# alibaba/VideoMV

Measured on AMD Instinct MI355X. Metric: denoise-steps/sec, t2v 320x512x24 (latent 24x40x64), CFG 9.0, 50-step DDIM schedule, higher is better.
Workload: dtype fp16; 1 GPU; t2v_infer.yaml UNetSD_T2VBase 1.413B, 24 views, latent 40x64, 77 ctx tokens, 1 sample per GPU (cond+uncond batched); parallelism=replicas x1

## Files before the change

videomv_amd/csrc/gemm_ff.hip:

```cpp
#include "gemm_glds_common.h"

using namespace vmvg;

namespace {

constexpr int FF_C = 320, FF_KS = FF_C / 32, FF_NT = FF_C / 16;
constexpr int FF_HC = 32;
constexpr int FF_W1_BYTES = 2 * FF_HC * FF_C * 2;
constexpr int FF_W2_BYTES = FF_C * FF_HC * 2;
constexpr int FF_STAGE = FF_W1_BYTES + FF_W2_BYTES;
constexpr int FF_B1_BYTES = 8 * FF_C * 4, FF_B2_BYTES = FF_C * 4;
constexpr int FF_LDS = 2 * FF_STAGE + FF_B1_BYTES + FF_B2_BYTES;
static_assert(FF_LDS <= 160 * 1024, "LDS budget");

constexpr int FF_PF1 = 1;
constexpr int FF_PF2 = 3;

VMV_DEV u32x4_t ff_swap16_xz_yw(u32x4_t v) {
    uint32_t x = v.x, y = v.y, z = v.z, w = v.w;
    asm("s_nop 3\n\tv_permlane16_swap_b32 %0, %2\n\tv_permlane16_swap_b32 %1, %3\n\ts_nop 1" : "+v"(x), "+v"(y), "+v"(z), "+v"(w));
    return u32x4_t{x, y, z, w};
}

__global__ __launch_bounds__(512, 1) void ff_fused_kernel(const VmvFfParams p) {
    VMV_KERNEL_ENTER();
    extern __shared__ __attribute__((aligned(16))) unsigned char smem[];
    const int tid = threadIdx.x;
    const int lane = tid & 63;
    const int wave = __builtin_amdgcn_readfirstlane(tid >> 6);
    const int frow = lane & 15, fgrp = lane >> 4;
    const int m_wave = blockIdx.x * 128 + wave * 16;
    const int nchunk = 4 * FF_C / FF_HC;

    const __amdgpu_buffer_rsrc_t x_rsrc = __builtin_amdgcn_make_buffer_rsrc(const_cast<void*>(p.x), 0, (uint32_t)p.M * (uint32_t)p.ldx * 2u, SRD_FLAGS);
    u32x4_t a[FF_KS];
    {
        const uint32_t vo = (uint32_t)((m_wave + frow) * p.ldx + 8 * fgrp) * 2u;
#pragma unroll
        for (int kk = 0; kk < FF_KS; ++kk) a[kk] = __builtin_amdgcn_raw_buffer_load_b128(x_rsrc, vo + (uint32_t)(kk * 64), 0, 0);
    }

    float* b1_lds = reinterpret_cast<float*>(smem + 2 * FF_STAGE);
    float* b2_lds = b1_lds + 8 * FF_C;
    {
        const __amdgpu_buffer_rsrc_t b1_rsrc = __builtin_amdgcn_make_buffer_rsrc(const_cast<float*>(p.b1), 0, p.b1 ? 8u * FF_C * 4u : 0u, SRD_FLAGS);
        const __amdgpu_buffer_rsrc_t b2_rsrc = __builtin_amdgcn_make_buffer_rsrc(const_cast<float*>(p.b2), 0, p.b2 ? FF_C * 4u : 0u, SRD_FLAGS);
        for (int q = wave; q * 256 < 8 * FF_C; q += 8)
            VMV_BLDS16(b1_rsrc, reinterpret_cast<unsigned char*>(b1_lds) + q * 1024, (uint32_t)(q * 256 + 4 * lane) * 4u, 0);
        if (wave < 2) VMV_BLDS16(b2_rsrc, reinterpret_cast<unsigned char*>(b2_lds) + wave * 1024, (uint32_t)(wave * 256 + 4 * lane) * 4u, 0);
    }
    const __amdgpu_buffer_rsrc_t w1_rsrc = __builtin_amdgcn_make_buffer_rsrc(const_cast<void*>(p.w1), 0, 8u * FF_C * FF_C * 2u, SRD_FLAGS);
    const __amdgpu_buffer_rsrc_t w2_rsrc = __builtin_amdgcn_make_buffer_rsrc(const_cast<void*>(p.w2), 0, (uint32_t)FF_C * 4u * FF_C * 2u, SRD_FLAGS);
    const int w2_slot = (lane & 3) ^ ((0x78 >> (2 * ((lane >> 4) & 3))) & 3);
    auto issue_chunk = [&](int c, int slot) {
        unsigned char* base = smem + slot * FF_STAGE;
        {
            const uint32_t so = (uint32_t)(c * 2 * FF_HC * FF_C) * 2u;
            int ln = lane;
            asm volatile("" : "+v"(ln));
#pragma unroll
            for (int q = 0; q < 5; ++q) {
                const int u = wave * 320 + q * 64 + ln;
                const int r = u / 40, s = u - r * 40;
                VMV_BLDS16(w1_rsrc, base + wave * 5120 + q * 1024, (uint32_t)(r * FF_C + (s ^ ((r >> 1) & 7)) * 8) * 2u, so);
            }
        }
        {
            const uint32_t so = (uint32_t)(c * FF_HC) * 2u;
            for (int t = wave; t < 20; t += 8)
                VMV_BLDS16(w2_rsrc, base + FF_W1_BYTES + t * 1024, (uint32_t)((16 * t + (lane >> 2)) * (4 * FF_C) + w2_slot * 8) * 2u, so);
        }
    };
    issue_chunk(0, 0);

    if (p.ln_eps > 0.f) {
        const float inv_k = 1.0f / (float)FF_C;
        float s1 = 0.f;
#pragma unroll
        for (int kk = 0; kk < FF_KS; ++kk) {
            elem_dot2c(s1, a[kk].x, VMV_ELEM_ONE2); elem_dot2c(s1, a[kk].y, VMV_ELEM_ONE2);
            elem_dot2c(s1, a[kk].z, VMV_ELEM_ONE2); elem_dot2c(s1, a[kk].w, VMV_ELEM_ONE2);
        }
        asm volatile("s_nop 4" : "+v"(s1));
        const float mean = xor16_32_sum(s1) * inv_k;
        float s2 = 0.f;
#pragma unroll
        for (int kk = 0; kk < FF_KS; ++kk) {
            const uint32_t w4[4] = {a[kk].x, a[kk].y, a[kk].z, a[kk].w};
#pragma unroll
            for (int e = 0; e < 4; ++e) {
                const float d0 = elem_lo(w4[e]) - mean, d1 = elem_hi(w4[e]) - mean;
                s2 = fmaf(d0, d0, s2); s2 = fmaf(d1, d1, s2);
            }
        }
        const float rstd = __builtin_amdgcn_rsqf(xor16_32_sum(s2) * inv_k + p.ln_eps);
        const float nm = -mean * rstd;
#pragma unroll
        for (int kk = 0; kk < FF_KS; ++kk) asm volatile("" : "+v"(a[kk].x), "+v"(a[kk].y), "+v"(a[kk].z), "+v"(a[kk].w));
#pragma unroll
        for (int kk = 0; kk < FF_KS; ++kk) {
            a[kk].x = pack_elem2(fmaf(elem_lo(a[kk].x), rstd, nm), fmaf(elem_hi(a[kk].x), rstd, nm));
            a[kk].y = pack_elem2(fmaf(elem_lo(a[kk].y), rstd, nm), fmaf(elem_hi(a[kk].y), rstd, nm));
            a[kk].z = pack_elem2(fmaf(elem_lo(a[kk].z), rstd, nm), fmaf(elem_hi(a[kk].z), rstd, nm));
            a[kk].w = pack_elem2(fmaf(elem_lo(a[kk].w), rstd, nm), fmaf(elem_hi(a[kk].w), rstd, nm));
        }
    }

    f32x4_t out[FF_NT];
#pragma unroll
    for (int j = 0; j < FF_NT; ++j) out[j] = f32x4_t{0.f, 0.f, 0.f, 0.f};

    const int fsw = (frow >> 1) & 7;
    int foff[2];
#pragma unroll
    for (int r = 0; r < 2; ++r) foff[r] = frow * 640 + (fgrp ^ (fsw & 3)) * 16 + ((r ^ (fsw >> 2)) - r) * 64;
    const int f2off = frow * 64 + (fgrp ^ ((0x78 >> (2 * ((frow >> 2) & 3))) & 3)) * 16;

    for (int c = 0; c < nchunk; ++c) {
        const int slot = c & 1;
        wait_vmcnt<0>();
        __builtin_amdgcn_s_waitcnt(0xc07f);
        __builtin_amdgcn_s_barrier();
        asm volatile("" ::: "memory");
        if (c + 1 < nchunk) issue_chunk(c + 1, slot ^ 1);
        const unsigned char* w1b = smem + slot * FF_STAGE;
        const unsigned char* w2b = w1b + FF_W1_BYTES + f2off;

        f32x4_t h1[4];
#pragma unroll
        for (int t = 0; t < 4; ++t) h1[t] = f32x4_t{0.f, 0.f, 0.f, 0.f};
        constexpr int PF1 = FF_PF1, NB1 = PF1 + 1;
        u32x4_t wf[NB1][4];
        auto rd1 = [&](const int kk, u32x4_t (&w)[4]) {
            const unsigned char* tp = w1b + foff[kk & 1] + 64 * kk;
#pragma unroll
            for (int t = 0; t < 4; ++t) w[t] = *reinterpret_cast<const u32x4_t*>(tp + t * (16 * 640));
        };
#pragma unroll
        for (int kk = 0; kk < PF1; ++kk) rd1(kk, wf[kk % NB1]);
#pragma unroll
        for (int kk = 0; kk < FF_KS; ++kk) {
            if (kk + PF1 < FF_KS) rd1(kk + PF1, wf[(kk + PF1) % NB1]);
            __builtin_amdgcn_sched_barrier(0);
#pragma unroll
            for (int t = 0; t < 4; ++t)
                h1[t] = VMV_MFMA16(__builtin_bit_cast(elem8_t, wf[kk % NB1][t]), __builtin_bit_cast(elem8_t, a[kk]), h1[t], 0, 0, 0);
            __builtin_amdgcn_sched_barrier(0);
        }
        constexpr int PF2 = FF_PF2, NB2 = PF2 + 1;
        u32x4_t w2f[NB2];
        auto rd2 = [&](const int j) -> u32x4_t { return *reinterpret_cast<const u32x4_t*>(w2b + j * (16 * 64)); };
#pragma unroll
        for (int j = 0; j < PF2; ++j) w2f[j % NB2] = rd2(j);
        u32x4_t hf;
        {
            const float* bb = b1_lds + c * 64 + 4 * fgrp;
            f32x4_t x0 = h1[0] + *reinterpret_cast<const f32x4_t*>(bb);
            const f32x4_t g0 = h1[1] + *reinterpret_cast<const f32x4_t*>(bb + 16);
            f32x4_t x1 = h1[2] + *reinterpret_cast<const f32x4_t*>(bb + 32);
            const f32x4_t g1 = h1[3] + *reinterpret_cast<const f32x4_t*>(bb + 48);
            x0.x *= gelu_erf_f(g0.x); x0.y *= gelu_erf_f(g0.y); x0.z *= gelu_erf_f(g0.z); x0.w *= gelu_erf_f(g0.w);
            x1.x *= gelu_erf_f(g1.x); x1.y *= gelu_erf_f(g1.y); x1.z *= gelu_erf_f(g1.z); x1.w *= gelu_erf_f(g1.w);
            hf.x = pack_elem2(x0.x, x0.y); hf.y = pack_elem2(x0.z, x0.w);
            hf.z = pack_elem2(x1.x, x1.y); hf.w = pack_elem2(x1.z, x1.w);
        }
#pragma unroll
        for (int j = 0; j < FF_NT; ++j) {
            if (j + PF2 < FF_NT) w2f[(j + PF2) % NB2] = rd2(j + PF2);
            __builtin_amdgcn_sched_barrier(0);
            out[j] = VMV_MFMA16(__builtin_bit_cast(elem8_t, w2f[j % NB2]), __builtin_bit_cast(elem8_t, hf), out[j], 0, 0, 0);
            __builtin_amdgcn_sched_barrier(0);
        }
    }

    const int lanecol = (fgrp & 1) * 16 + (fgrp >> 1) * 8;
    const __amdgpu_buffer_rsrc_t out_rsrc = __builtin_amdgcn_make_buffer_rsrc(p.out, 0, SRD_RECORDS, SRD_FLAGS);
    const __amdgpu_buffer_rsrc_t res_rsrc = __builtin_amdgcn_make_buffer_rsrc(const_cast<void*>(p.residual), 0, SRD_RECORDS, SRD_FLAGS);
    const bool ok = m_wave + frow < p.M;
    const uint32_t ovo = ok ? (uint32_t)((m_wave + frow) * p.ldo + lanecol) * 2u : OOB;
    const uint32_t rvo = (ok && p.residual) ? (uint32_t)((m_wave + frow) * p.ldr + lanecol) * 2u : OOB;
#pragma unroll
    for (int jp = 0; jp < FF_NT / 2; ++jp) {
        const u32x4_t rr = ff_swap16_xz_yw(__builtin_amdgcn_raw_buffer_load_b128(res_rsrc, rvo, (uint32_t)(32 * jp) * 2u, 0));
        f32x4_t v0 = out[2 * jp] + *reinterpret_cast<const f32x4_t*>(b2_lds + 32 * jp + 4 * fgrp);
        f32x4_t v1 = out[2 * jp + 1] + *reinterpret_cast<const f32x4_t*>(b2_lds + 32 * jp + 16 + 4 * fgrp);
        v0.x += elem_lo(rr.x); v0.y += elem_hi(rr.x); v0.z += elem_lo(rr.y); v0.w += elem_hi(rr.y);
        v1.x += elem_lo(rr.z); v1.y += elem_hi(rr.z); v1.z += elem_lo(rr.w); v1.w += elem_hi(rr.w);
        u32x4_t o;
        o.x = pack_elem2(v0.x, v0.y); o.y = pack_elem2(v0.z, v0.w);
        o.z = pack_elem2(v1.x, v1.y); o.w = pack_elem2(v1.z, v1.w);
        o = ff_swap16_xz_yw(o);
        __builtin_amdgcn_raw_buffer_store_b128(o, out_rsrc, ovo, (uint32_t)(32 * jp) * 2u, 0);
        asm volatile("s_nop 7" ::"v"(o.x), "v"(o.y), "v"(o.z), "v"(o.w) : "memory");
    }
}

}

extern "C" int vmv_ff_fused_ok(const VmvFfParams* pp) {
    if (!pp) return 0;
    const VmvFfParams& p = *pp;
    if (p.C != FF_C || p.M <= 0 || !p.x || !p.w1 || !p.w2 || !p.out) return 0;
    if ((p.ldx & 7) || (p.ldo & 7) || (p.residual && (p.ldr & 7))) return 0;
    if (!vmv_aligned16(p.x) || !vmv_aligned16(p.w1) || !vmv_aligned16(p.w2) || !vmv_aligned16(p.out) || (p.residual && !vmv_aligned16(p.residual))) return 0;
    if ((p.b1 && !vmv_aligned16(p.b1)) || (p.b2 && !vmv_aligned16(p.b2))) return 0;
    if ((long)(p.M + 128) * p.ldx * 2 >= (1L << 31) - 65536 || (long)(p.M + 128) * p.ldo * 2 >= (1L << 31) - 65536) return 0;
    if (p.residual && (long)(p.M + 128) * p.ldr * 2 >= (1L << 31) - 65536) return 0;
    return 1;
}

extern "C" int vmv_ff_fused(const VmvFfParams* pp, void* stream) {
    if (!pp) return VMV_ENULL;
    const VmvFfParams& p = *pp;
    if (!p.x || !p.w1 || !p.w2 || !p.out) return VMV_ENULL;
    if (p.C != FF_C || p.M <= 0) return VMV_EINVAL;
    if (!vmv_ff_fused_ok(pp)) return VMV_EALIGN;
    static std::atomic<unsigned long long> attr{0};
    if (const int rc_attr = vmv_lds_attr_once(attr, reinterpret_cast<const void*>(&ff_fused_kernel), FF_LDS)) return rc_attr;
    hipLaunchKernelGGL(ff_fused_kernel, dim3((p.M + 127) / 128), dim3(512), FF_LDS, reinterpret_cast<hipStream_t>(stream), p);
    return vmv_launch_status();
}
```

videomv_amd/unet_engine.py:

```python
import ctypes as C
import math
import os
from typing import Dict, List, Optional

import torch

from . import _lib as L
from . import ops
from . import packing as P



def block_plan(cfg):
    dim = cfg["dim"]
    dim_mult = list(cfg["dim_mult"])
    nrb = cfg["num_res_blocks"]
    hd = cfg["head_dim"]
    attn_scales = list(cfg["attn_scales"])
    enc_dims = [dim * u for u in [1] + dim_mult]
    dec_dims = [dim * u for u in [dim_mult[-1]] + dim_mult[::-1]]
    shortcut, scale = [], 1.0
    inp = [[("conv_in", "input_blocks.0.0", dict(cin=cfg["in_dim"], cout=dim)),
            ("tt", "input_blocks.0.1", dict(c=dim, heads=cfg["num_heads"], dh=hd))]]
    shortcut.append(dim)
    idx, out_dim = 1, dim
    for i, (in_dim, out_dim) in enumerate(zip(enc_dims[:-1], enc_dims[1:])):
        for j in range(nrb):
            p = f"input_blocks.{idx}"
            blk = [("res", f"{p}.0", dict(cin=in_dim, cout=out_dim))]
            if scale in attn_scales:
                blk.append(("st", f"{p}.1", dict(c=out_dim, heads=out_dim // hd, dh=hd, ctx=cfg["context_dim"])))
                blk.append(("tt", f"{p}.2", dict(c=out_dim, heads=out_dim // hd, dh=hd)))
            in_dim = out_dim
            inp.append(blk)
            shortcut.append(out_dim)
            idx += 1
            if i != len(dim_mult) - 1 and j == nrb - 1:
                inp.append([("down", f"input_blocks.{idx}", dict(c=out_dim))])
                shortcut.append(out_dim)
                scale /= 2.0
                idx += 1
    mid = [("res", "middle_block.0", dict(cin=out_dim, cout=out_dim)),
           ("st", "middle_block.1", dict(c=out_dim, heads=out_dim // hd, dh=hd, ctx=cfg["context_dim"])),
           ("tt", "middle_block.2", dict(c=out_dim, heads=out_dim // hd, dh=hd)),
           ("res", "middle_block.3", dict(cin=out_dim, cout=out_dim))]
    outb, idx = [], 0
    for i, (in_dim, out_dim) in enumerate(zip(dec_dims[:-1], dec_dims[1:])):
        for j in range(nrb + 1):
            p = f"output_blocks.{idx}"
            sc = shortcut.pop()
            blk = [("res", f"{p}.0", dict(cin=in_dim + sc, cout=out_dim, c_main=in_dim, c_skip=sc))]
            k = 1
            if scale in attn_scales:
                blk.append(("st", f"{p}.{k}", dict(c=out_dim, heads=out_dim // hd, dh=hd, ctx=1024)))
                blk.append(("tt", f"{p}.{k + 1}", dict(c=out_dim, heads=out_dim // hd, dh=hd)))
                k += 2
            in_dim = out_dim
            if i != len(dim_mult) - 1 and j == nrb:
                blk.append(("up", f"{p}.{k}", dict(c=out_dim)))
                scale *= 2.0
            outb.append(blk)
            idx += 1
    return inp, mid, outb


def _attn_shapes(p, c, inner, ctx):
    kv = inner if ctx is None else ctx
    return [(f"{p}.to_q.weight", (inner, c)), (f"{p}.to_k.weight", (inner, kv)), (f"{p}.to_v.weight", (inner, kv)),
            (f"{p}.to_out.0.weight", (c, inner)), (f"{p}.to_out.0.bias", (c,))]


def _tblock_shapes(p, inner, ctx):
    s = _attn_shapes(f"{p}.attn1", inner, inner, None)
    s += [(f"{p}.ff.net.0.proj.weight", (inner * 8, inner)), (f"{p}.ff.net.0.proj.bias", (inner * 8,)),
          (f"{p}.ff.net.2.weight", (inner, inner * 4)), (f"{p}.ff.net.2.bias", (inner,))]
    s += _attn_shapes(f"{p}.attn2", inner, inner, ctx)
    for n in ("norm1", "norm2", "norm3"):
        s += [(f"{p}.{n}.weight", (inner,)), (f"{p}.{n}.bias", (inner,))]
    return s


def param_shapes(cfg) -> "Dict[str, tuple]":
    dim = cfg["dim"]
    E = dim * 4
    s = [("time_embed.0.weight", (E, dim)), ("time_embed.0.bias", (E,)),
         ("time_embed.2.weight", (E, E)), ("time_embed.2.bias", (E,))]
    if cfg.get("use_camera_condition", False):
        s += [("camera_embedding.0.weight", (E, cfg["camera_dim"])), ("camera_embedding.0.bias", (E,)),
              ("camera_embedding.2.weight", (E, E)), ("camera_embedding.2.bias", (E,))]
    if cfg.get("use_fps_condition", False):
        s += [("fps_embedding.0.weight", (E, dim)), ("fps_embedding.0.bias", (E,)),
              ("fps_embedding.2.weight", (E, E)), ("fps_embedding.2.bias", (E,))]
    inp, mid, outb = block_plan(cfg)
    for blk in inp + [mid] + outb:
        for kind, p, m in blk:
            if kind == "conv_in":
                s += [(f"{p}.weight", (m["cout"], m["cin"], 3, 3)), (f"{p}.bias", (m["cout"],))]
            elif kind == "res":
                ci, co = m["cin"], m["cout"]
                s += [(f"{p}.in_layers.0.weight", (ci,)), (f"{p}.in_layers.0.bias", (ci,)),
                      (f"{p}.in_layers.2.weight", (co, ci, 3, 3)), (f"{p}.in_layers.2.bias", (co,)),
                      (f"{p}.emb_layers.1.weight", (co, E)), (f"{p}.emb_layers.1.bias", (co,)),
                      (f"{p}.out_layers.0.weight", (co,)), (f"{p}.out_layers.0.bias", (co,)),
                      (f"{p}.out_layers.3.weight", (co, co, 3, 3)), (f"{p}.out_layers.3.bias", (co,))]
                if ci != co:
                    s += [(f"{p}.skip_connection.weight", (co, ci, 1, 1)), (f"{p}.skip_connection.bias", (co,))]
                for name, ix in (("conv1", 2), ("conv2", 3), ("conv3", 3), ("conv4", 3)):
                    q = f"{p}.temopral_conv.{name}"
                    s += [(f"{q}.0.weight", (co,)), (f"{q}.0.bias", (co,)),
                          (f"{q}.{ix}.weight", (co, co, 3, 1, 1)), (f"{q}.{ix}.bias", (co,))]
            elif kind in ("st", "tt"):
                c = m["c"]
                inner = m["heads"] * m["dh"]
                s += [(f"{p}.norm.weight", (c,)), (f"{p}.norm.bias", (c,))]
                if kind == "st":
                    s += [(f"{p}.proj_in.weight", (inner, c)), (f"{p}.proj_in.bias", (inner,))]
                    s += _tblock_shapes(f"{p}.transformer_blocks.0", inner, m["ctx"])
                    s += [(f"{p}.proj_out.weight", (inner, c)), (f"{p}.proj_out.bias", (inner,))]
                else:
                    s += [(f"{p}.proj_in.weight", (inner, c, 1)), (f"{p}.proj_in.bias", (inner,))]
                    s += _tblock_shapes(f"{p}.transformer_blocks.0", inner, None)
                    s += [(f"{p}.proj_out.weight", (c, inner, 1)), (f"{p}.proj_out.bias", (c,))]
            elif kind == "down":
                s += [(f"{p}.op.weight", (m["c"], m["c"], 3, 3)), (f"{p}.op.bias", (m["c"],))]
            elif kind == "up":
                s += [(f"{p}.conv.weight", (m["c"], m["c"], 3, 3)), (f"{p}.conv.bias", (m["c"],))]
    s += [("out.0.weight", (dim,)), ("out.0.bias", (dim,)),
          ("out.2.weight", (cfg["out_dim"], dim, 3, 3)), ("out.2.bias", (cfg["out_dim"],))]
    return dict(s)


class Pool:

    def __init__(self, device):
        self.device = device
        self.free: Dict[int, List[torch.Tensor]] = {}
        self.all: List[torch.Tensor] = []
        self.bytes = 0

    def get(self, nbytes: int) -> torch.Tensor:
        nbytes = (int(nbytes) + 255) // 256 * 256
        lst = self.free.get(nbytes)
        if lst:
            return lst.pop()
        t = torch.empty(nbytes, dtype=torch.uint8, device=self.device)
        self.all.append(t)
        self.bytes += nbytes
        return t

    def put(self, t: torch.Tensor):
        self.free.setdefault(t.numel(), []).append(t)


class Act:
    __slots__ = ("buf", "rows", "C", "dtype")

    def __init__(self, buf, rows, C, dtype=None):
        self.buf, self.rows, self.C, self.dtype = buf, rows, C, dtype or L.elem()

    @property
    def ptr(self):
        return self.buf.data_ptr()

    def tensor(self) -> torch.Tensor:
        esz = 4 if self.dtype == torch.float32 else 2
        return self.buf[: self.rows * self.C * esz].view(self.dtype).view(self.rows, self.C)


class UNetEngine:
    def __init__(self, cfg: dict, weights: Dict[str, torch.Tensor], B: int, F: int, H: int, W: int, L_ctx: int,
                 device, n_t: int = 1, taps: Optional[dict] = None, comm=None, share_prefix: bool = False,
                 packed: Optional[dict] = None, eps_out: Optional[torch.Tensor] = None):
        self.share_prefix = bool(share_prefix) and B >= 2 and B % 2 == 0 and n_t == 1 and comm is None
        self.Bp = B // 2 if self.share_prefix else B
        self.comm = comm
        self.R = comm.world if comm is not None else 1
        self.rk = comm.rank if comm is not None else 0
        self.Fg = F
        if F % self.R:
            raise ValueError(f"{F} frames do not split over {self.R} ranks")
        F = F // self.R
        self.cfg, self.B, self.F, self.H, self.W, self.L = cfg, B, F, H, W, L_ctx
        self.B_ctx = B
        self.device = device
        self.breaks = []
        self.n_comm_ops, self.comm_bytes_in = 0, 0
        self.pool = Pool(device)
        self.S = ops.Stream(record=True)
        self.Sctx = ops.Stream(record=True)
        self._keepalive = []
        self._splitk = None
        self._gnws = torch.empty(4 << 20, dtype=torch.float32, device=device)
        self._gn_tot2 = torch.zeros(2, B * ops.GN_TOT, dtype=torch.int64, device=device)
        self._gn_zero = torch.zeros(2, B * ops.GN_TOT, dtype=torch.int64, device=device)
        self._gn_tot_k = 0
        self._gn_tot_all = torch.zeros(B * ops.GN_TOT * self.R, dtype=torch.int64, device=device) if comm is not None else None
        self.taps = taps
        self.n_t = n_t
        self.dim = cfg["dim"]
        self.E = self.dim * 4
        self.inp, self.mid, self.outb = block_plan(cfg)
        self.fold_ln = os.environ.get("VMV_FOLD_LN", "1") != "0"
        self.ln_inline = os.environ.get("VMV_LN_INLINE", "0") == "1"
        self.ff_fused = os.environ.get("VMV_FF_FUSED", "0") == "1" and self.fold_ln
        self.tqa = os.environ.get("VMV_TQA", "1") != "0"
        self.use_graph, self._replays, self.graph_nodes = os.environ.get("VMV_GRAPH", "0") == "1", 0, 0
        self.fp_temporal = os.environ.get("VMV_FP_TEMPORAL", "switch")
        if self.fp_temporal not in ("switch", "kv_gather"):
            raise ValueError("VMV_FP_TEMPORAL must be 'switch' or 'kv_gather'")
        if packed is not None and packed.get("fold_ln") == self.fold_ln and packed.get("device") == str(device):
            for k, v in packed.items():
                if k not in ("fold_ln", "device"):
                    setattr(self, k, v)
        else:
            self._pack(weights)
        self.packed = dict(fold_ln=self.fold_ln, device=str(device), w=self.w, has_cam=self.has_cam, has_fps=self.has_fps,
                           emb_off=self.emb_off, emb_total=self.emb_total, out_pad=self.out_pad)
        self._eps_out = eps_out
        self.n_tuned, self.n_ruled, self.n_stale = 0, 0, 0
        self.S.tuner = ops.make_tuner(self)
        self._static_inputs()
        self._build()
        if os.environ.get("VMV_AUTOTUNE", "0") == "1" and taps is None and str(device).startswith("cuda"):
            from . import autotune
            if autotune.autotune_engine(self, tag=f"B{B} F{self.Fg} {H}x{W} world{self.R}") > 0:
                self._rerecord()

    def _rerecord(self):
        dev = self.device
        self.B = self.B_ctx
        self.breaks, self.n_comm_ops, self.comm_bytes_in = [], 0, 0
        self.pool = Pool(dev)
        self.S = ops.Stream(record=True)
        self.Sctx = ops.Stream(record=True)
        self._keepalive, self._splitk = [], None
        self._gn_tot2.zero_()
        self._gn_tot_k = 0
        self._replays, self.graph_nodes, self.n_tuned, self.n_ruled, self.n_stale = 0, 0, 0, 0, 0
        self.S.tuner = ops.make_tuner(self)
        self._static_inputs()
        self._build()

    def _pack(self, sd):
        dev = self.device
        w: Dict[str, torch.Tensor] = {}
        self.w = w

        def lin(key, bias=True):
            w[key + ".weight"] = P.pack_linear(sd[key + ".weight"], dev)
            if bias and (key + ".bias") in sd:
                w[key + ".bias"] = P.pack_bias(sd[key + ".bias"], dev)

        def norm(key):
            w[key + ".weight"] = P.f32(sd[key + ".weight"], dev)
            w[key + ".bias"] = P.f32(sd[key + ".bias"], dev)

        def folded(key, wt, b, nkey, geglu=False):
            if not self.fold_ln:
                return
            wf, bf, cs = P.fold_layernorm(wt, b, sd[nkey + ".weight"], sd[nkey + ".bias"])
            if geglu:
                wf, bf, cs = P.geglu_interleave(wf), P.geglu_interleave(bf), P.geglu_interleave(cs)
            w[key + ".ln.weight"] = P.pack_linear(wf, dev)
            w[key + ".ln.bias"] = P.pack_bias(bf, dev)
            w[key + ".ln.colsum"] = P.pack_bias(cs, dev)

        def tblock(p, temporal=False):
            for a in ("attn1", "attn2"):
                q = sd[f"{p}.{a}.to_q.weight"]
                k = sd[f"{p}.{a}.to_k.weight"]
                v = sd[f"{p}.{a}.to_v.weight"]
                nk = "norm1" if a == "attn1" else "norm2"
                if k.shape[1] == q.shape[1]:
                    if not self.fold_ln:
                        w[f"{p}.{a}.qkv"] = P.pack_linear(torch.cat([q, k, v], dim=0), dev)
                    folded(f"{p}.{a}.qkv", torch.cat([q, k, v], dim=0), None, f"{p}.{nk}")
                    if temporal and self.tqa and q.shape[1] == 320 and q.shape[0] % 64 == 0:
                        for sfx in ((".ln.weight", ".ln.bias", ".ln.colsum") if self.fold_ln else ("",)):
                            src = w[f"{p}.{a}.qkv{sfx}"]
                            w[f"{p}.{a}.qkv.hm{sfx}"] = P.qkv_head_major(src[: 3 * q.shape[0]]).contiguous()
                else:
                    if not self.fold_ln:
                        w[f"{p}.{a}.q"] = P.pack_linear(q, dev)
                    folded(f"{p}.{a}.q", q, None, f"{p}.{nk}")
                    w[f"{p}.{a}.kv"] = P.pack_linear(torch.cat([k, v], dim=0), dev)
                lin(f"{p}.{a}.to_out.0")
            if not self.fold_ln:
                w[f"{p}.ff.net.0.proj.weight"] = P.pack_linear(P.geglu_interleave(sd[f"{p}.ff.net.0.proj.weight"]), dev)
            w[f"{p}.ff.net.0.proj.bias"] = P.pack_bias(P.geglu_interleave(sd[f"{p}.ff.net.0.proj.bias"]), dev)
            folded(f"{p}.ff.net.0.proj", sd[f"{p}.ff.net.0.proj.weight"], sd[f"{p}.ff.net.0.proj.bias"], f"{p}.norm3", geglu=True)
            lin(f"{p}.ff.net.2")
            if self.fold_ln and sd[f"{p}.ff.net.2.weight"].shape[0] == 320:
                w[f"{p}.ff.net.2.weight.ffperm"] = P.pack_linear(P.ff_down_permute(sd[f"{p}.ff.net.2.weight"]), dev)
            for n in ("norm1", "norm2", "norm3"):
                norm(f"{p}.{n}")

        lin("time_embed.0"); lin("time_embed.2")
        self.has_cam = "camera_embedding.0.weight" in sd
        if self.has_cam:
            lin("camera_embedding.0"); lin("camera_embedding.2")
        self.has_fps = self.cfg.get("use_fps_condition", False) and "fps_embedding.0.weight" in sd
        if self.has_fps:
            lin("fps_embedding.0"); lin("fps_embedding.2")
        emb_w, emb_b, self.emb_off = [], [], {}
        off = 0
        for blk in self.inp + [self.mid] + self.outb:
            for kind, p, m in blk:
                if kind == "conv_in":
                    w[p + ".weight"] = P.pack_conv3x3(sd[p + ".weight"], dev)
                    w[p + ".bias"] = P.pack_bias(sd[p + ".bias"], dev)
                elif kind == "res":
                    norm(f"{p}.in_layers.0")
                    w[f"{p}.in_layers.2.weight"] = P.pack_conv3x3(sd[f"{p}.in_layers.2.weight"], dev)
                    w[f"{p}.in_layers.2.bias"] = P.pack_bias(sd[f"{p}.in_layers.2.bias"], dev)
                    emb_w.append(sd[f"{p}.emb_layers.1.weight"]); emb_b.append(sd[f"{p}.emb_layers.1.bias"])
                    self.emb_off[p] = off
                    off += m["cout"]
                    norm(f"{p}.out_layers.0")
                    w2 = sd[f"{p}.out_layers.3.weight"]
# ... 253 lines not shown
        T = B * F * h * w
        cout = m["cout"]
        geom = ops.Geom(OH=h, OW=w, IH=h, IW=w, stride=1, ups=0)
        h0 = self._gn(p + ".gn1", srcs, T, h * w, f"{p}.in_layers.0", 1e-5, True)
        h1 = self.act(T, cout)
        self._gemm(p + ".conv1", T, cout, ops.conv3x3_segs([(h0.ptr, h0.C, h0.C)]), f"{p}.in_layers.2.weight", h1,
                   bias=self.w[f"{p}.in_layers.2.bias"], geom=geom,
                   rowvec=self.emb_out.data_ptr() + 4 * self.emb_off[p], rowvec_div=h * w, rowvec_ld=self.emb_total)
        self.release(h0)
        h2 = self._gn(p + ".gn2", [h1], T, h * w, f"{p}.out_layers.0", 1e-5, True)
        self.release(h1)
        h3 = self.act(T, cout)
        segs = ops.conv3x3_segs([(h2.ptr, h2.C, h2.C)])
        if m["cin"] != cout:
            segs += ops.linear_segs([(s.ptr, s.C, s.C) for s in srcs])
            self._gemm(p + ".conv2+skip", T, cout, segs, f"{p}.conv2.weight", h3, bias=self.w[f"{p}.conv2.bias"], geom=geom)
        else:
            self._gemm(p + ".conv2", T, cout, segs, f"{p}.conv2.weight", h3, bias=self.w[f"{p}.conv2.bias"], geom=geom,
                       residual=srcs[0].ptr, ldr=srcs[0].C)
        self.release(h2)
        if self.comm is not None:
            h3 = self._switch(h3, h * w, to_pixel=True)
        tg = ops.Geom(F=self.Fg, P=(h * w) // self.R)
        cur = h3
        for i, name in enumerate(("conv1", "conv2", "conv3", "conv4")):
            q = f"{p}.temopral_conv.{name}"
            nxt = self.act(T, cout)
            last = i == 3
            if not self._tconv_folded(q, cur, T, F * h * w, nxt, tg, residual=h3.ptr if last else None, ldr=h3.C if last else 0):
                g = self._gn(q + ".gn", [cur], T, F * h * w, f"{q}.0", 1e-5, True, all_frames=True)
                self._gemm(q, T, cout, ops.temporal_segs(g.ptr, g.C, g.C), f"{q}.weight", nxt, bias=self.w[f"{q}.bias"],
                           geom=tg, residual=h3.ptr if last else None, ldr=h3.C if last else 0)
                self.release(g)
            if cur is not h3:
                self.release(cur)
            cur = nxt
        self.release(h3)
        if self.comm is not None:
            cur = self._switch(cur, h * w, to_pixel=False)
        return cur

    def _tblock(self, p, a: Act, heads, temporal: bool, h, w, cross_ctx: bool, phase: str = "all", kv_gather: bool = False) -> Act:
        B, F = self.B, self.F
        T = a.rows
        inner = a.C
        hw = h * w
        scale = 64 ** -0.5

        if temporal and not kv_gather:
            hw, F = hw // self.R, self.Fg

        def maps(ld, col0=0):
            if temporal:
                return ops.seq_map(F * hw * ld, ld, hw * ld, inner=hw)
            return ops.seq_map(hw * ld, 0, ld, inner=1)

        n_outer = B * hw if temporal else B * F
        Nq = F if temporal else hw

        def fused_qkv_attn(tag, x: Act, normkey):
            hm = f"{p}.{tag}.qkv.hm"
            if not (temporal and not kv_gather and self.tqa and (hm + (".ln.weight" if self.fold_ln else "")) in self.w):
                return None
            ao = self.act(T, inner)
            geom = ops.Geom(F=F, P=hw)
            if self.fold_ln:
                gp = ops.gemm_params(T, 3 * inner, ops.linear_segs([(x.ptr, x.C, x.C)]), self.w[hm + ".ln.weight"], ao.ptr, ao.C,
                                     bias=self.w[hm + ".ln.bias"], colsum=self.w[hm + ".ln.colsum"], ln_eps=1e-5,
                                     epilogue=L.EPI_TATTN, epi_scale=scale, geom=geom)
                ln = None
            else:
                ln = self._ln(f"{p}.{tag}.qkv.ln", x, f"{p}.{normkey}")
                gp = ops.gemm_params(T, 3 * inner, ops.linear_segs([(ln.ptr, ln.C, ln.C)]), self.w[hm], ao.ptr, ao.C,
                                     epilogue=L.EPI_TATTN, epi_scale=scale, geom=geom)
            if not self.S.lib.vmv_gemm_tqa_ok(C.byref(gp)):
                self.release(ao)
                if ln is not None:
                    self.release(ln)
                return None
            self.S.gemm(gp, f"{p}.{tag}.qkv+attn")
            if ln is not None:
                self.release(ln)
            return ao

        def self_attn(tag, x: Act, normkey) -> Act:
            ao = fused_qkv_attn(tag, x, normkey)
            if ao is not None:
                y = self.act(T, inner)
                self._gemm(f"{p}.{tag}.out", T, inner, ops.linear_segs([(ao.ptr, ao.C, ao.C)]), f"{p}.{tag}.to_out.0.weight", y,
                           bias=self.w[f"{p}.{tag}.to_out.0.bias"], residual=x.ptr, ldr=x.C)
                self.release(ao)
                return y
            qkv = self.act(T, 3 * inner)
            self._ln_linear(f"{p}.{tag}.qkv", x, f"{p}.{normkey}", 3 * inner, f"{p}.{tag}.qkv", qkv)
            ao = self.act(T, inner)
            ld = 3 * inner
            if kv_gather:
                cv = inner // 8
                kvloc = self.act(T, 2 * inner)
                self.S.copy(ops.copy_params(qkv.ptr + 2 * inner, kvloc.ptr, T, 1, 1, 2 * cv, 3 * cv, 0), f"{p}.{tag}.kv.pack")
                kvall = self.act(self.R * T, 2 * inner)
                out_t, in_t = kvall.tensor().view(-1), kvloc.tensor().view(-1)
                self._collective(L.COMM_ALL_GATHER, out_t, in_t, f"{p}.{tag}.kv.gather")
                self.release(kvloc)
                qm = ops.seq_map(0, ld, hw * ld, inner=hw)
                km = ops.seq_map(0, 2 * inner, hw * 2 * inner, inner=hw)
                self.S.attention(ops.attn_params(qkv.ptr, kvall.ptr, kvall.ptr + 2 * inner, ao.ptr, qm, km, km,
                                                 ops.seq_map(0, inner, hw * inner, inner=hw), hw, heads, F, self.Fg, scale),
                                 f"{p}.{tag}.attn")
                self.release(kvall)
            else:
                self.S.attention(ops.attn_params(qkv.ptr, qkv.ptr + 2 * inner, qkv.ptr + 4 * inner, ao.ptr,
                                                 maps(ld), maps(ld), maps(ld), maps(inner), n_outer, heads, Nq, Nq, scale),
                                 f"{p}.{tag}.attn")
            self.release(qkv)
            y = self.act(T, inner)
            self._gemm(f"{p}.{tag}.out", T, inner, ops.linear_segs([(ao.ptr, ao.C, ao.C)]), f"{p}.{tag}.to_out.0.weight", y,
                       bias=self.w[f"{p}.{tag}.to_out.0.bias"], residual=x.ptr, ldr=x.C)
            self.release(ao)
            return y

        def cross_attn(tag, x: Act, normkey) -> Act:
            q = self.act(T, inner)
            self._ln_linear(f"{p}.{tag}.q", x, f"{p}.{normkey}", inner, f"{p}.{tag}.q", q)
            Lc = self.L
            Bc = self.B_ctx
            kvt = torch.empty(Bc * Lc, 2 * inner, dtype=L.elem(), device=self.device)
            self._keepalive.append(kvt)
            kv = Act(kvt.view(torch.uint8).view(-1), Bc * Lc, 2 * inner)
            cd = self.ctx_rows.shape[1]
            self._gemm(f"{p}.{tag}.kv", Bc * Lc, 2 * inner, ops.linear_segs([(self.ctx_rows.data_ptr(), cd, cd)]),
                       f"{p}.{tag}.kv", kv, stream=self.Sctx)
            ao = self.act(T, inner)
            kvm = ops.seq_map(Lc * 2 * inner, 0, 2 * inner, inner=1)
            self.S.attention(ops.attn_params(q.ptr, kv.ptr, kv.ptr + 2 * inner, ao.ptr, maps(inner), kvm, kvm, maps(inner),
                                             n_outer, heads, Nq, Lc, scale, kv_div=F), f"{p}.{tag}.attn")
            self.release(q)
            y = self.act(T, inner)
            self._gemm(f"{p}.{tag}.out", T, inner, ops.linear_segs([(ao.ptr, ao.C, ao.C)]), f"{p}.{tag}.to_out.0.weight", y,
                       bias=self.w[f"{p}.{tag}.to_out.0.bias"], residual=x.ptr, ldr=x.C)
            self.release(ao)
            return y

        if phase == "post":
            a1 = a
        else:
            a1 = self_attn("attn1", a, "norm1")
            if phase == "pre":
                return a1
        a2 = cross_attn("attn2", a1, "norm2") if cross_ctx else self_attn("attn2", a1, "norm2")
        if phase != "post":
            self.release(a1)
        a3 = self.act(T, inner)
        if self.ff_fused and f"{p}.ff.net.2.weight.ffperm" in self.w and T >= 16384:
            fp = ops.ff_params(T, inner, a2.ptr, a2.C, self.w[f"{p}.ff.net.0.proj.ln.weight"], self.w[f"{p}.ff.net.0.proj.ln.bias"],
                               self.w[f"{p}.ff.net.2.weight.ffperm"], self.w[f"{p}.ff.net.2.bias"], a3.ptr, a3.C,
                               residual=a2.ptr, ldr=a2.C, ln_eps=1e-5)
            if self.S.lib.vmv_ff_fused_ok(C.byref(fp)):
                self.S.ff(fp, f"{p}.ff.fused")
                self.release(a2)
                return a3
        ff = self.act(T, 4 * inner)
        self._ln_linear(f"{p}.ff.geglu", a2, f"{p}.norm3", 8 * inner, f"{p}.ff.net.0.proj.weight", ff,
                        bias=self.w[f"{p}.ff.net.0.proj.bias"], epilogue=L.EPI_GEGLU)
        self._gemm(f"{p}.ff.down", T, inner, ops.linear_segs([(ff.ptr, ff.C, ff.C)]), f"{p}.ff.net.2.weight", a3,
                   bias=self.w[f"{p}.ff.net.2.bias"], residual=a2.ptr, ldr=a2.C)
        self.release(ff); self.release(a2)
        return a3

    def _transformer(self, kind, p, m, x: Act, h, w, cut: bool = False) -> Act:
        B, F = self.B, self.F
        T = x.rows
        C = x.C
        inner = m["heads"] * m["dh"]
        if m["dh"] != 64:
            raise NotImplementedError("the HIP attention kernel is specialised for head_dim 64")
        temporal = kind == "tt"
        sharded = temporal and self.comm is not None
        kvg = sharded and self.fp_temporal == "kv_gather" and self.B == 1 and not cut
        if sharded and not kvg:
            x = self._switch(x, h * w, to_pixel=True, release_in=False)
        rps = (F * h * w) if temporal else (h * w)
        a = self.act(T, inner)
        if not self._gn_folded_proj_in(p, x, T, rps, a, temporal):
            n0 = self._gn(p + ".norm", [x], T, rps, f"{p}.norm", 1e-6, False, all_frames=temporal)
            self._gemm(p + ".proj_in", T, inner, ops.linear_segs([(n0.ptr, n0.C, n0.C)]), f"{p}.proj_in.weight", a,
                       bias=self.w[f"{p}.proj_in.bias"])
            self.release(n0)
        if cut:
            assert not temporal and self.B == self.Bp
            a1 = self._tblock(f"{p}.transformer_blocks.0", a, m["heads"], temporal, h, w, cross_ctx=True, phase="pre")
            self.release(a)
            self.B = self.B_ctx
            x_full, a1_full = self._replicate(x, p + ".share.x"), self._replicate(a1, p + ".share.a1")
            self.release(a1)
            x, T = x_full, x_full.rows
            a3 = self._tblock(f"{p}.transformer_blocks.0", a1_full, m["heads"], temporal, h, w, cross_ctx=True, phase="post")
            self.release(a1_full)
        else:
            a3 = self._tblock(f"{p}.transformer_blocks.0", a, m["heads"], temporal, h, w, cross_ctx=not temporal, kv_gather=kvg)
            self.release(a)
        y = self.act(T, C)
        self._gemm(p + ".proj_out", T, C, ops.linear_segs([(a3.ptr, a3.C, a3.C)]), f"{p}.proj_out.weight", y,
                   bias=self.w[f"{p}.proj_out.bias"], residual=x.ptr, ldr=x.C)
        self.release(a3)
        if cut:
            self.release(x)
        if sharded and not kvg:
            self.release(x)
            y = self._switch(y, h * w, to_pixel=False)
        return y

    def _run_block(self, blk, srcs: List[Act], h, w):
        x = None
        for kind, p, m in blk:
            ins = srcs if x is None else [x]
            if kind == "conv_in":
                T_in = self.B * self.F * h * w
                y = self.act(T_in, m["cout"])
                self._gemm(p, T_in, m["cout"], ops.conv3x3_segs([(self.x_rows.data_ptr(), self.cin_pad, self.cin_pad)]),
                           p + ".weight", y, bias=self.w[p + ".bias"], geom=ops.Geom(OH=h, OW=w, IH=h, IW=w))
            elif kind == "res":
                y = self._res_block(p, m, ins, h, w)
            elif kind in ("st", "tt"):
                y = self._transformer(kind, p, m, ins[0], h, w, cut=(kind == "st" and self.B != self.B_ctx))
            elif kind == "down":
                xin = ins[0]
                oh, ow = (h + 1) // 2, (w + 1) // 2
                T = self.B * self.F * oh * ow
                y = self.act(T, m["c"])
                self._gemm(p, T, m["c"], ops.conv3x3_segs([(xin.ptr, xin.C, xin.C)]), p + ".weight", y,
                           bias=self.w[p + ".bias"], geom=ops.Geom(OH=oh, OW=ow, IH=h, IW=w, stride=2))
                h, w = oh, ow
            elif kind == "up":
                xin = ins[0]
                oh, ow = h * 2, w * 2
                T = self.B * self.F * oh * ow
                y = self.act(T, m["c"])
                self._gemm(p, T, m["c"], ops.conv3x3_segs([(xin.ptr, xin.C, xin.C)]), p + ".weight", y,
                           bias=self.w[p + ".bias"], geom=ops.Geom(OH=oh, OW=ow, IH=h, IW=w, stride=1, ups=1))
                h, w = oh, ow
            else:
                raise ValueError(kind)
            if x is not None:
                self.release(x)
            x = y
        return x, h, w

    def _build(self):
        B, F = self.B, self.F
        S = self.S
        S.copy(ops.copy_params(self._gn_zero.data_ptr(), self._gn_tot2.data_ptr(), 1, 1, 1, self._gn_tot2.numel() // 2, 0, 0),
               "gn.totals.clear")
        self.n_emb_ops_start = S.nops
        e = Act(self.emb_silu.view(torch.uint8).view(-1), B * F, self.E)
        eo = Act(self.emb_out.view(torch.uint8).view(-1), B * F, self.emb_total, torch.float32)
        self._gemm("emb_all", B * F, self.emb_total, ops.linear_segs([(e.ptr, e.C, e.C)]), "emb_all.weight", eo,
                   bias=self.w["emb_all.bias"], out_fp32=True)
        h, w = self.H, self.W
        xs = []
        x = None
        share = self.share_prefix and len(self.inp) > 1 and any(k == "st" for k, _, _ in self.inp[1])
        if share:
            self.B = self.Bp
        for bi, blk in enumerate(self.inp):
            x, h, w = self._run_block(blk, [x] if x is not None else [], h, w)
            if share and bi == 0:
                x1 = x
                x_skip = self._replicate(x1, "share.skip0")
                xs.append((x_skip, h, w))
                if self.taps is not None:
                    self.taps[blk[0][1]] = (x_skip, h, w)
                continue
            if share and bi == 1:
                self.release(x1)
            xs.append((x, h, w))
            if self.taps is not None:
                self.taps[blk[0][1]] = (x, h, w)
        assert self.B == self.B_ctx
        x_last = x
        x, h, w = self._run_block(self.mid, [x], h, w)
        if self.taps is not None:
            self.taps["middle_block"] = (x, h, w)
        for blk in self.outb:
            skip, sh, sw = xs.pop()
            assert (sh, sw) == (h, w), (sh, sw, h, w)
            y, h, w = self._run_block(blk, [x, skip], h, w)
            if x is not skip:
                self.release(x)
            self.release(skip)
            x = y
            if self.taps is not None:
                self.taps[blk[0][1]] = (x, h, w)
        T = self.T0
        hn = self._gn("out.gn", [x], T, h * w, "out.0", 1e-5, True)
        self.release(x)
        eps = Act(self.eps_rows.view(torch.uint8).view(-1), T, self.out_pad, torch.float32)
        self._gemm("out.conv", T, self.out_pad, ops.conv3x3_segs([(hn.ptr, hn.C, hn.C)]), "out.2.weight", eps,
                   bias=self.w["out.2.bias"], geom=ops.Geom(OH=h, OW=w, IH=h, IW=w), out_fp32=True)
        self.release(hn)

    def set_context(self, y: torch.Tensor):
        self.ctx_rows.copy_(y.reshape(self.B * self.L, -1).to(L.elem()))
        self.context_updated()

    def context_updated(self):
        if self.Sctx.nops:
# ... 133 lines not shown
```

Baseline: 19.73 denoise-steps/s.

## Split fused FF wave work across wave pairs with software-pipelined down-projection

```diff
diff --git a/videomv_amd/csrc/gemm_ff.hip b/videomv_amd/csrc/gemm_ff.hip
--- a/videomv_amd/csrc/gemm_ff.hip
+++ b/videomv_amd/csrc/gemm_ff.hip
@@ -8,12 +8,14 @@
 constexpr int FF_HC = 32;
 constexpr int FF_W1_BYTES = 2 * FF_HC * FF_C * 2;
 constexpr int FF_W2_BYTES = FF_C * FF_HC * 2;
-constexpr int FF_STAGE = FF_W1_BYTES + FF_W2_BYTES;
-constexpr int FF_B1_BYTES = 8 * FF_C * 4, FF_B2_BYTES = FF_C * 4;
-constexpr int FF_LDS = 2 * FF_STAGE + FF_B1_BYTES + FF_B2_BYTES;
+constexpr int FF_B1_PIECE = 1024, FF_B2_BYTES = FF_C * 4;
+constexpr int FF_XCH_BYTES = 8 * 2 * 512;
+constexpr int FF_OFF_W2 = 2 * FF_W1_BYTES, FF_OFF_B1 = FF_OFF_W2 + 3 * FF_W2_BYTES, FF_OFF_B2 = FF_OFF_B1 + 2 * FF_B1_PIECE;
+constexpr int FF_OFF_XCH = FF_OFF_B2 + FF_B2_BYTES;
+constexpr int FF_LDS = FF_OFF_XCH + 2 * FF_XCH_BYTES;
 static_assert(FF_LDS <= 160 * 1024, "LDS budget");
 
-constexpr int FF_PF1 = 1;
+constexpr int FF_PF1 = 2;
 constexpr int FF_PF2 = 3;
 
 VMV_DEV u32x4_t ff_swap16_xz_yw(u32x4_t v) {
@@ -29,51 +31,50 @@
     const int lane = tid & 63;
     const int wave = __builtin_amdgcn_readfirstlane(tid >> 6);
     const int frow = lane & 15, fgrp = lane >> 4;
-    const int m_wave = blockIdx.x * 128 + wave * 16;
+    const int m_wave = blockIdx.x * 128 + (wave >> 1) * 32;
+    const int half = wave & 1;
     const int nchunk = 4 * FF_C / FF_HC;
 
     const __amdgpu_buffer_rsrc_t x_rsrc = __builtin_amdgcn_make_buffer_rsrc(const_cast<void*>(p.x), 0, (uint32_t)p.M * (uint32_t)p.ldx * 2u, SRD_FLAGS);
-    u32x4_t a[FF_KS];
+    u32x4_t a[2][FF_KS];
     {
-        const uint32_t vo = (uint32_t)((m_wave + frow) * p.ldx + 8 * fgrp) * 2u;
-#pragma unroll
-        for (int kk = 0; kk < FF_KS; ++kk) a[kk] = __builtin_amdgcn_raw_buffer_load_b128(x_rsrc, vo + (uint32_t)(kk * 64), 0, 0);
-    }
-
-    float* b1_lds = reinterpret_cast<float*>(smem + 2 * FF_STAGE);
-    float* b2_lds = b1_lds + 8 * FF_C;
+#pragma unroll
+        for (int rt = 0; rt < 2; ++rt) {
+        const uint32_t vo = (uint32_t)((m_wave + 16 * rt + frow) * p.ldx + 8 * fgrp) * 2u;
+#pragma unroll
+        for (int kk = 0; kk < FF_KS; ++kk) a[rt][kk] = __builtin_amdgcn_raw_buffer_load_b128(x_rsrc, vo + (uint32_t)(kk * 64), 0, 0);
+        }
+    }
+
+    float* b2_lds = reinterpret_cast<float*>(smem + FF_OFF_B2);
     {
-        const __amdgpu_buffer_rsrc_t b1_rsrc = __builtin_amdgcn_make_buffer_rsrc(const_cast<float*>(p.b1), 0, p.b1 ? 8u * FF_C * 4u : 0u, SRD_FLAGS);
         const __amdgpu_buffer_rsrc_t b2_rsrc = __builtin_amdgcn_make_buffer_rsrc(const_cast<float*>(p.b2), 0, p.b2 ? FF_C * 4u : 0u, SRD_FLAGS);
-        for (int q = wave; q * 256 < 8 * FF_C; q += 8)
-            VMV_BLDS16(b1_rsrc, reinterpret_cast<unsigned char*>(b1_lds) + q * 1024, (uint32_t)(q * 256 + 4 * lane) * 4u, 0);
         if (wave < 2) VMV_BLDS16(b2_rsrc, reinterpret_cast<unsigned char*>(b2_lds) + wave * 1024, (uint32_t)(wave * 256 + 4 * lane) * 4u, 0);
     }
+    const __amdgpu_buffer_rsrc_t b1_rsrc = __builtin_amdgcn_make_buffer_rsrc(const_cast<float*>(p.b1), 0, p.b1 ? 8u * FF_C * 4u : 0u, SRD_FLAGS);
     const __amdgpu_buffer_rsrc_t w1_rsrc = __builtin_amdgcn_make_buffer_rsrc(const_cast<void*>(p.w1), 0, 8u * FF_C * FF_C * 2u, SRD_FLAGS);
     const __amdgpu_buffer_rsrc_t w2_rsrc = __builtin_amdgcn_make_buffer_rsrc(const_cast<void*>(p.w2), 0, (uint32_t)FF_C * 4u * FF_C * 2u, SRD_FLAGS);
     const int w2_slot = (lane & 3) ^ ((0x78 >> (2 * ((lane >> 4) & 3))) & 3);
-    auto issue_chunk = [&](int c, int slot) {
-        unsigned char* base = smem + slot * FF_STAGE;
-        {
-            const uint32_t so = (uint32_t)(c * 2 * FF_HC * FF_C) * 2u;
-            int ln = lane;
-            asm volatile("" : "+v"(ln));
-#pragma unroll
-            for (int q = 0; q < 5; ++q) {
-                const int u = wave * 320 + q * 64 + ln;
-                const int r = u / 40, s = u - r * 40;
-                VMV_BLDS16(w1_rsrc, base + wave * 5120 + q * 1024, (uint32_t)(r * FF_C + (s ^ ((r >> 1) & 7)) * 8) * 2u, so);
-            }
-        }
-        {
-            const uint32_t so = (uint32_t)(c * FF_HC) * 2u;
-            for (int t = wave; t < 20; t += 8)
-                VMV_BLDS16(w2_rsrc, base + FF_W1_BYTES + t * 1024, (uint32_t)((16 * t + (lane >> 2)) * (4 * FF_C) + w2_slot * 8) * 2u, so);
-        }
-    };
-    issue_chunk(0, 0);
-
-    if (p.ln_eps > 0.f) {
+    uint32_t v1off[5], v2off = (uint32_t)((lane >> 2) * (4 * FF_C) + w2_slot * 8) * 2u;
+#pragma unroll
+    for (int q = 0; q < 5; ++q) {
+        const int u = wave * 320 + q * 64 + lane;
+        const int r = u / 40, s = u - r * 40;
+        v1off[q] = (uint32_t)(r * FF_C + (s ^ ((r >> 1) & 7)) * 8) * 2u;
+        asm volatile("" : "+v"(v1off[q]));
+    }
+    asm volatile("" : "+v"(v2off));
+    auto issue_chunk = [&](const int c, const int s1, const int s2) {
+#pragma unroll
+        for (int q = 0; q < 5; ++q)
+            VMV_BLDS16(w1_rsrc, smem + s1 * FF_W1_BYTES + wave * 5120 + q * 1024, v1off[q], (uint32_t)(c * 2 * FF_HC * FF_C) * 2u);
+        for (int t = wave; t < 20; t += 8)
+            VMV_BLDS16(w2_rsrc, smem + FF_OFF_W2 + s2 * FF_W2_BYTES + t * 1024, v2off, (uint32_t)(16 * t * (4 * FF_C) + c * FF_HC) * 2u);
+        if (wave == 7) VMV_BLDS16(b1_rsrc, smem + FF_OFF_B1 + s1 * FF_B1_PIECE, (uint32_t)(c * 256 + lane * 16), 0);
+    };
+    issue_chunk(0, 0, 0);
+
+    auto lnorm = [&](u32x4_t (&a)[FF_KS]) {
         const float inv_k = 1.0f / (float)FF_C;
         float s1 = 0.f;
 #pragma unroll
@@ -104,37 +105,83 @@
             a[kk].z = pack_elem2(fmaf(elem_lo(a[kk].z), rstd, nm), fmaf(elem_hi(a[kk].z), rstd, nm));
             a[kk].w = pack_elem2(fmaf(elem_lo(a[kk].w), rstd, nm), fmaf(elem_hi(a[kk].w), rstd, nm));
         }
-    }
-
-    f32x4_t out[FF_NT];
-#pragma unroll
-    for (int j = 0; j < FF_NT; ++j) out[j] = f32x4_t{0.f, 0.f, 0.f, 0.f};
-
+    };
+    if (p.ln_eps > 0.f) { lnorm(a[0]); lnorm(a[1]); }
+
+
+    f32x4_t out[2][FF_NT / 2];
+#pragma unroll
+    for (int rt = 0; rt < 2; ++rt)
+#pragma unroll
+        for (int j = 0; j < FF_NT / 2; ++j) out[rt][j] = f32x4_t{0.f, 0.f, 0.f, 0.f};
     const int fsw = (frow >> 1) & 7;
     int foff[2];
 #pragma unroll
     for (int r = 0; r < 2; ++r) foff[r] = frow * 640 + (fgrp ^ (fsw & 3)) * 16 + ((r ^ (fsw >> 2)) - r) * 64;
     const int f2off = frow * 64 + (fgrp ^ ((0x78 >> (2 * ((frow >> 2) & 3))) & 3)) * 16;
-
-    for (int c = 0; c < nchunk; ++c) {
-        const int slot = c & 1;
+    unsigned char* xch = smem + FF_OFF_XCH;
+
+    f32x4_t h1[2][2];
+    constexpr int PF2 = FF_PF2, NB2 = PF2 + 1;
+    u32x4_t w2f[NB2], hf[2];
+    const unsigned char* w2b = smem;
+    auto rd2 = [&](const int j) -> u32x4_t { return *reinterpret_cast<const u32x4_t*>(w2b + j * (16 * 64)); };
+    auto ff2_fetch = [&](const int d, const int s2) {
+        const unsigned char* xb = xch + (d & 1) * FF_XCH_BYTES + (wave & ~1) * 1024 + lane * 8;
+#pragma unroll
+        for (int rt = 0; rt < 2; ++rt) {
+            const uint2 lo = *reinterpret_cast<const uint2*>(xb + rt * 512), hi = *reinterpret_cast<const uint2*>(xb + 1024 + rt * 512);
+            hf[rt] = u32x4_t{lo.x, lo.y, hi.x, hi.y};
+        }
+        w2b = smem + FF_OFF_W2 + s2 * FF_W2_BYTES + f2off + half * (10 * 16 * 64);
+#pragma unroll
+        for (int j = 0; j < PF2; ++j) w2f[j % NB2] = rd2(j);
+    };
+    auto geglu = [&](const int c) {
+        const float* bb = reinterpret_cast<const float*>(smem + FF_OFF_B1 + (c & 1) * FF_B1_PIECE) + 32 * half + 4 * fgrp;
+        const f32x4_t bx = *reinterpret_cast<const f32x4_t*>(bb), bg = *reinterpret_cast<const f32x4_t*>(bb + 16);
+#pragma unroll
+        for (int rt = 0; rt < 2; ++rt) {
+            f32x4_t x0 = h1[rt][0] + bx;
+            const f32x4_t g0 = h1[rt][1] + bg;
+            x0.x *= gelu_erf_f(g0.x); x0.y *= gelu_erf_f(g0.y); x0.z *= gelu_erf_f(g0.z); x0.w *= gelu_erf_f(g0.w);
+            *reinterpret_cast<uint2*>(xch + (c & 1) * FF_XCH_BYTES + wave * 1024 + rt * 512 + lane * 8) = uint2{pack_elem2(x0.x, x0.y), pack_elem2(x0.z, x0.w)};
+        }
+    };
+    auto ff2_mma = [&]() {
+#pragma unroll
+        for (int j = 0; j < FF_NT / 2; ++j) {
+            if (j + PF2 < FF_NT / 2) w2f[(j + PF2) % NB2] = rd2(j + PF2);
+            __builtin_amdgcn_sched_barrier(0);
+#pragma unroll
+            for (int rt = 0; rt < 2; ++rt)
+                out[rt][j] = VMV_MFMA16(__builtin_bit_cast(elem8_t, w2f[j % NB2]), __builtin_bit_cast(elem8_t, hf[rt]), out[rt][j], 0, 0, 0);
+            __builtin_amdgcn_sched_barrier(0);
+        }
+    };
+    auto rendezvous = [&]() {
         wait_vmcnt<0>();
         __builtin_amdgcn_s_waitcnt(0xc07f);
         __builtin_amdgcn_s_barrier();
         asm volatile("" ::: "memory");
-        if (c + 1 < nchunk) issue_chunk(c + 1, slot ^ 1);
-        const unsigned char* w1b = smem + slot * FF_STAGE;
-        const unsigned char* w2b = w1b + FF_W1_BYTES + f2off;
-
-        f32x4_t h1[4];
-#pragma unroll
-        for (int t = 0; t < 4; ++t) h1[t] = f32x4_t{0.f, 0.f, 0.f, 0.f};
+    };
+
+    int s2p = 2, s2c = 0;
+    for (int c = 0; c < nchunk; ++c) {
+        rendezvous();
+        const int s2n = s2c == 2 ? 0 : s2c + 1;
+        if (c + 1 < nchunk) issue_chunk(c + 1, (c + 1) & 1, s2n);
+        const unsigned char* w1b = smem + (c & 1) * FF_W1_BYTES + half * (32 * 640);
+#pragma unroll
+        for (int rt = 0; rt < 2; ++rt)
+#pragma unroll
+            for (int t = 0; t < 2; ++t) h1[rt][t] = f32x4_t{0.f, 0.f, 0.f, 0.f};
         constexpr int PF1 = FF_PF1, NB1 = PF1 + 1;
-        u32x4_t wf[NB1][4];
-        auto rd1 = [&](const int kk, u32x4_t (&w)[4]) {
+        u32x4_t wf[NB1][2];
+        auto rd1 = [&](const int kk, u32x4_t (&w)[2]) {
             const unsigned char* tp = w1b + foff[kk & 1] + 64 * kk;
 #pragma unroll
-            for (int t = 0; t < 4; ++t) w[t] = *reinterpret_cast<const u32x4_t*>(tp + t * (16 * 640));
+            for (int t = 0; t < 2; ++t) w[t] = *reinterpret_cast<const u32x4_t*>(tp + t * (16 * 640));
         };
 #pragma unroll
         for (int kk = 0; kk < PF1; ++kk) rd1(kk, wf[kk % NB1]);
@@ -143,47 +190,35 @@
             if (kk + PF1 < FF_KS) rd1(kk + PF1, wf[(kk + PF1) % NB1]);
             __builtin_amdgcn_sched_barrier(0);
 #pragma unroll
-            for (int t = 0; t < 4; ++t)
-                h1[t] = VMV_MFMA16(__builtin_bit_cast(elem8_t, wf[kk % NB1][t]), __builtin_bit_cast(elem8_t, a[kk]), h1[t], 0, 0, 0);
-            __builtin_amdgcn_sched_barrier(0);
-        }
-        constexpr int PF2 = FF_PF2, NB2 = PF2 + 1;
-        u32x4_t w2f[NB2];
-        auto rd2 = [&](const int j) -> u32x4_t { return *reinterpret_cast<const u32x4_t*>(w2b + j * (16 * 64)); };
-#pragma unroll
-        for (int j = 0; j < PF2; ++j) w2f[j % NB2] = rd2(j);
-        u32x4_t hf;
-        {
-            const float* bb = b1_lds + c * 64 + 4 * fgrp;
-            f32x4_t x0 = h1[0] + *reinterpret_cast<const f32x4_t*>(bb);
-            const f32x4_t g0 = h1[1] + *reinterpret_cast<const f32x4_t*>(bb + 16);
-            f32x4_t x1 = h1[2] + *reinterpret_cast<const f32x4_t*>(bb + 32);
-            const f32x4_t g1 = h1[3] + *reinterpret_cast<const f32x4_t*>(bb + 48);
-            x0.x *= gelu_erf_f(g0.x); x0.y *= gelu_erf_f(g0.y); x0.z *= gelu_erf_f(g0.z); x0.w *= gelu_erf_f(g0.w);
-            x1.x *= gelu_erf_f(g1.x); x1.y *= gelu_erf_f(g1.y); x1.z *= gelu_erf_f(g1.z); x1.w *= gelu_erf_f(g1.w);
-            hf.x = pack_elem2(x0.x, x0.y); hf.y = pack_elem2(x0.z, x0.w);
-            hf.z = pack_elem2(x1.x, x1.y); hf.w = pack_elem2(x1.z, x1.w);
-        }
-#pragma unroll
-        for (int j = 0; j < FF_NT; ++j) {
-            if (j + PF2 < FF_NT) w2f[(j + PF2) % NB2] = rd2(j + PF2);
-            __builtin_amdgcn_sched_barrier(0);
-            out[j] = VMV_MFMA16(__builtin_bit_cast(elem8_t, w2f[j % NB2]), __builtin_bit_cast(elem8_t, hf), out[j], 0, 0, 0);
-            __builtin_amdgcn_sched_barrier(0);
-        }
-    }
-
-    const int lanecol = (fgrp & 1) * 16 + (fgrp >> 1) * 8;
+            for (int t = 0; t < 2; ++t)
+#pragma unroll
+                for (int rt = 0; rt < 2; ++rt)
+                    h1[rt][t] = VMV_MFMA16(__builtin_bit_cast(elem8_t, wf[kk % NB1][t]), __builtin_bit_cast(elem8_t, a[rt][kk]), h1[rt][t], 0, 0, 0);
+            __builtin_amdgcn_sched_barrier(0);
+        }
+        if (c > 0) ff2_fetch(c - 1, s2p);
+        geglu(c);
+        __builtin_amdgcn_sched_barrier(0);
+        if (c > 0) ff2_mma();
+        s2p = s2c; s2c = s2n;
+    }
+    rendezvous();
+    ff2_fetch(nchunk - 1, s2p);
+    ff2_mma();
+
+    const int lanecol = 160 * half + (fgrp & 1) * 16 + (fgrp >> 1) * 8;
     const __amdgpu_buffer_rsrc_t out_rsrc = __builtin_amdgcn_make_buffer_rsrc(p.out, 0, SRD_RECORDS, SRD_FLAGS);
     const __amdgpu_buffer_rsrc_t res_rsrc = __builtin_amdgcn_make_buffer_rsrc(const_cast<void*>(p.residual), 0, SRD_RECORDS, SRD_FLAGS);
-    const bool ok = m_wave + frow < p.M;
-    const uint32_t ovo = ok ? (uint32_t)((m_wave + frow) * p.ldo + lanecol) * 2u : OOB;
-    const uint32_t rvo = (ok && p.residual) ? (uint32_t)((m_wave + frow) * p.ldr + lanecol) * 2u : OOB;
-#pragma unroll
-    for (int jp = 0; jp < FF_NT / 2; ++jp) {
+#pragma unroll
+    for (int rt = 0; rt < 2; ++rt) {
+    const bool ok = m_wave + 16 * rt + frow < p.M;
+    const uint32_t ovo = ok ? (uint32_t)((m_wave + 16 * rt + frow) * p.ldo + lanecol) * 2u : OOB;
+    const uint32_t rvo = (ok && p.residual) ? (uint32_t)((m_wave + 16 * rt + frow) * p.ldr + lanecol) * 2u : OOB;
+#pragma unroll
+    for (int jp = 0; jp < FF_NT / 4; ++jp) {
         const u32x4_t rr = ff_swap16_xz_yw(__builtin_amdgcn_raw_buffer_load_b128(res_rsrc, rvo, (uint32_t)(32 * jp) * 2u, 0));
-        f32x4_t v0 = out[2 * jp] + *reinterpret_cast<const f32x4_t*>(b2_lds + 32 * jp + 4 * fgrp);
-        f32x4_t v1 = out[2 * jp + 1] + *reinterpret_cast<const f32x4_t*>(b2_lds + 32 * jp + 16 + 4 * fgrp);
+        f32x4_t v0 = out[rt][2 * jp] + *reinterpret_cast<const f32x4_t*>(b2_lds + 160 * half + 32 * jp + 4 * fgrp);
+        f32x4_t v1 = out[rt][2 * jp + 1] + *reinterpret_cast<const f32x4_t*>(b2_lds + 160 * half + 32 * jp + 16 + 4 * fgrp);
         v0.x += elem_lo(rr.x); v0.y += elem_hi(rr.x); v0.z += elem_lo(rr.y); v0.w += elem_hi(rr.y);
         v1.x += elem_lo(rr.z); v1.y += elem_hi(rr.z); v1.z += elem_lo(rr.w); v1.w += elem_hi(rr.w);
         u32x4_t o;
@@ -192,6 +227,7 @@
         o = ff_swap16_xz_yw(o);
         __builtin_amdgcn_raw_buffer_store_b128(o, out_rsrc, ovo, (uint32_t)(32 * jp) * 2u, 0);
         asm volatile("s_nop 7" ::"v"(o.x), "v"(o.y), "v"(o.z), "v"(o.w) : "memory");
+    }
     }
 }
 
diff --git a/videomv_amd/unet_engine.py b/videomv_amd/unet_engine.py
--- a/videomv_amd/unet_engine.py
+++ b/videomv_amd/unet_engine.py
@@ -165,6 +165,12 @@
     def tensor(self) -> torch.Tensor:
         esz = 4 if self.dtype == torch.float32 else 2
         return self.buf[: self.rows * self.C * esz].view(self.dtype).view(self.rows, self.C)
+
+
+def _ff_fused_rows(T: int) -> bool:
+    blocks = (T + 127) // 128
+    rounds = (blocks + 255) // 256
+    return T >= 16384 and 8 * (256 * rounds - blocks) <= 256 * rounds
 
 
 class UNetEngine:
@@ -724,7 +730,7 @@
         if phase != "post":
             self.release(a1)
         a3 = self.act(T, inner)
-        if self.ff_fused and f"{p}.ff.net.2.weight.ffperm" in self.w and T >= 16384:
+        if self.ff_fused and f"{p}.ff.net.2.weight.ffperm" in self.w and _ff_fused_rows(T):
             fp = ops.ff_params(T, inner, a2.ptr, a2.C, self.w[f"{p}.ff.net.0.proj.ln.weight"], self.w[f"{p}.ff.net.0.proj.ln.bias"],
                                self.w[f"{p}.ff.net.2.weight.ffperm"], self.w[f"{p}.ff.net.2.bias"], a3.ptr, a3.C,
                                residual=a2.ptr, ldr=a2.C, ln_eps=1e-5)
```

New measurement: 19.65 denoise-steps/s. No clear change (-0.4%).
